# MOLAorg/mola_lidar_odometry

Hardware: AMD Instinct MI355X
Metric: scans/sec (KITTI 64-beam, ~120k pts, 1M-pt map) @1/2/4/8 GPU; ATE vs ref (higher is better)
Workload: dtype f32 points / f64 accumulators

## Files before the change

### mola_lidar_odometry_amd/csrc/mh_k_launch.h

```cpp
#pragma once

__global__ __launch_bounds__(kBlock, MH_QUAD_WAVES) void k_match4(const IcpDeviceState* __restrict__ st,
                                                   const float* __restrict__ lx, const float* __restrict__ ly,
                                                   const float* __restrict__ lz, uint32_t n, MapView map,
                                                   float4* __restrict__ pair_q, uint32_t* __restrict__ pair_gidx,
                                                   const uint32_t* __restrict__ perm
#ifdef MH_DEBUG_WAVETRACE
                                                   , unsigned long long* __restrict__ wtrace
#endif
) {
  k_match4_body(st, lx, ly, lz, n, map, pair_q, pair_gidx, perm
#ifdef MH_DEBUG_WAVETRACE
                , wtrace
#endif
  );
}
#ifndef MH_FLAT_WAVES
#define MH_FLAT_WAVES 6
#endif
#ifndef MH_FLAT_THREADS
#define MH_FLAT_THREADS 64
#endif
constexpr uint32_t kFlatThreads = MH_FLAT_THREADS;
constexpr uint32_t kFlatPointsPerBlock = kFlatThreads;
__device__ __forceinline__ uint32_t nblk_flat_dev(uint32_t n) { return (n + kFlatPointsPerBlock - 1u) / kFlatPointsPerBlock; }
constexpr uint32_t kFlatGridUnit = 8u;
inline uint32_t nblk_flat(size_t n) { return (uint32_t)(((n + kFlatPointsPerBlock - 1) / kFlatPointsPerBlock + kFlatGridUnit - 1) / kFlatGridUnit * kFlatGridUnit); }
__device__ __forceinline__ void k_match_flat_body(const IcpDeviceState* __restrict__ st, const float* __restrict__ lx,
                                                  const float* __restrict__ ly, const float* __restrict__ lz, uint32_t n,
                                                  MapView map, float4* __restrict__ pair_q, uint32_t* __restrict__ pair_gidx,
                                                  const uint32_t* __restrict__ perm, uint32_t block_x) {
  __shared__ FlatWave sh[kFlatThreads / 64];
  typedef const IcpDeviceState __attribute__((address_space(4))) * cstate_ptr;
  const cstate_ptr cst = (cstate_ptr)uniform_const_ptr(st);
  if (cst->done) return;
  const uint32_t bx = block_x;
  const uint32_t i0 = bx * kFlatPointsPerBlock + (threadIdx.x & ~63u);
  if (i0 >= n) return;
  const bool have_prev = cst->iter > 0 && !map.no_prev_bound;
  double T[12];
#pragma unroll
  for (int k = 0; k < 12; k++) T[k] = cst->T[k];
  match_flat_wave(sh[threadIdx.x >> 6], map, T, cst->cur_thr2, cst->cur_ang2, have_prev, lx, ly, lz, n, i0, pair_q, pair_gidx, perm);
}
__global__ __launch_bounds__(kFlatThreads, MH_FLAT_WAVES) void k_match_flat(const IcpDeviceState* __restrict__ st, const float* __restrict__ lx,
                                                             const float* __restrict__ ly, const float* __restrict__ lz, uint32_t n,
                                                             MapView map, float4* __restrict__ pair_q,
                                                             uint32_t* __restrict__ pair_gidx, const uint32_t* __restrict__ perm) {
  k_match_flat_body(st, lx, ly, lz, n, map, pair_q, pair_gidx, perm, blockIdx.x);
}
__global__ __launch_bounds__(kBlock, MH_QUAD_WAVES) void k_match4_b(const BatchJob* __restrict__ jobs) {
  const BatchJob& j = jobs[blockIdx.y];
  k_match4_body(j.st, j.lx, j.ly, j.lz, j.n, j.map, j.pair_q, j.pair_gidx, nullptr
#ifdef MH_DEBUG_WAVETRACE
                , nullptr
#endif
  );
}
__global__ __launch_bounds__(kFlatThreads, MH_FLAT_WAVES) void k_match_flat_b(const BatchJob* __restrict__ jobs) {
  uint32_t job = blockIdx.y, bx = blockIdx.x;
  const uint32_t whole = gridDim.y & ~7u;
  if (blockIdx.y < whole) {
    const uint32_t L = blockIdx.x + blockIdx.y * gridDim.x, xcd = L % 8u, slot = L / 8u;
    job = xcd + 8u * (slot / gridDim.x);
    bx = slot % gridDim.x;
  }
  const BatchJob& j = jobs[job];
  k_match_flat_body(j.st, j.lx, j.ly, j.lz, j.n, j.map, j.pair_q, j.pair_gidx, nullptr, bx);
}
#ifdef MH_DEV_VARIANTS
#include "mh_dev_variants.h"
#endif
template <bool SIGNED>
__global__ __launch_bounds__(kBlock, MH_ACCUM_WAVES) void k_accum(const IcpDeviceState* __restrict__ st, uint32_t first,
                                                  const MatchK* __restrict__ kp, const float* __restrict__ lx,
                                                  const float* __restrict__ ly, const float* __restrict__ lz, uint32_t n,
                                                  const float4* __restrict__ pair_q,
                                                  const uint32_t* __restrict__ pair_gidx, double* __restrict__ partials,
                                                  uint32_t pstride) {
  k_accum_body<SIGNED>(st, first, kp, lx, ly, lz, n, pair_q, pair_gidx, partials, pstride, blockIdx.x);
}
template <bool SIGNED>
__global__ __launch_bounds__(kBlock, MH_ACCUM_WAVES) void k_accum_b(const BatchJob* __restrict__ jobs, uint32_t first) {
  const BatchJob& j = jobs[blockIdx.y];
  const uint32_t bx = blockIdx.x;
  if (bx >= j.nba) return;
  k_accum_body<SIGNED>(j.st, first, j.mk, j.lx, j.ly, j.lz, j.n, j.pair_q, j.pair_gidx, j.part, j.nba, bx);
}
__global__ __launch_bounds__(kSolveThreads) void k_solve(IcpDeviceState* __restrict__ st, const SolveK* __restrict__ kp,
                                                         const double* __restrict__ partA, uint32_t nA, uint32_t strideA,
                                                         const double* __restrict__ partB, uint32_t nB,
                                                         uint32_t strideB, uint32_t first) {
  k_solve_body(st, kp, partA, nA, strideA, partB, nB, strideB, first);
}
__global__ __launch_bounds__(kSolveThreads) void k_solve_b(const BatchJob* __restrict__ jobs, uint32_t first) {
  const BatchJob& j = jobs[blockIdx.y];
  const uint32_t cols = first ? j.nbm : j.nba;
  k_solve_body(j.st, j.sk, j.part, cols, cols, nullptr, 0u, 0u, first);
}
__global__ void k_cov_prepare(IcpDeviceState* __restrict__ st, const SolveK* __restrict__ kp, uint32_t force) {
  k_cov_prepare_body(st, kp, force);
}
__global__ void k_cov_prepare_b(const BatchJob* __restrict__ jobs) {
  const BatchJob& j = jobs[blockIdx.y];
  k_cov_prepare_body(j.st, j.sk, 0u);
}
__global__ __launch_bounds__(kBlock) void k_cov_accum(const IcpDeviceState* __restrict__ st, uint32_t force,
                                                      const float* __restrict__ lx, const float* __restrict__ ly,
                                                      const float* __restrict__ lz, uint32_t n,
                                                      const uint32_t* __restrict__ pair_gidx,
                                                      double* __restrict__ partials, uint32_t pstride) {
  k_cov_accum_body(st, force, lx, ly, lz, n, pair_gidx, partials, pstride, blockIdx.x);
}
__global__ __launch_bounds__(kBlock) void k_cov_accum_b(const BatchJob* __restrict__ jobs) {
  const BatchJob& j = jobs[blockIdx.y];
  if (blockIdx.x >= j.nb) return;
  k_cov_accum_body(j.st, 0u, j.lx, j.ly, j.lz, j.n, j.pair_gidx, j.part, j.nb, blockIdx.x);
}
__global__ __launch_bounds__(kSolveThreads) void k_cov_finalize(IcpDeviceState* __restrict__ st, uint32_t force,
                                                                const double* __restrict__ partA, uint32_t nA,
                                                                uint32_t strideA, const double* __restrict__ partB,
                                                                uint32_t nB, uint32_t strideB) {
  k_cov_finalize_body(st, force, partA, nA, strideA, partB, nB, strideB);
}
__global__ __launch_bounds__(kSolveThreads) void k_cov_finalize_b(const BatchJob* __restrict__ jobs) {
  const BatchJob& j = jobs[blockIdx.y];
// ... 34 lines not shown
```

### mola_lidar_odometry_amd/csrc/mh_k_layers.h

```cpp
#pragma once

struct LayerDesc {
  MapView map;
  const float *lx, *ly, *lz;
  float4* pair_q;
  uint32_t* pair_gidx;
  MatchK mk;
  uint32_t n;
  uint32_t col_off;
  uint32_t cov_off;
  uint32_t run_from;
  uint32_t run_up_to;
  uint32_t kpp;
};

struct LayerTable {
  uint32_t n_pairs, pad;
  uint32_t blk_match[MH_MAX_LAYER_PAIRS + 1];
  uint32_t blk_acc[MH_MAX_LAYER_PAIRS + 1];
  uint32_t blk_cov[MH_MAX_LAYER_PAIRS + 1];
  LayerDesc d[MH_MAX_LAYER_PAIRS];
};

typedef const LayerTable __attribute__((address_space(4))) * clayers_ptr;

__device__ __forceinline__ uint32_t layer_of(const uint32_t __attribute__((address_space(4))) * start, uint32_t np, uint32_t b) {
  uint32_t li = 0;
  for (uint32_t k = 1; k < np; k++) li += b >= start[k] ? 1u : 0u;
  return li;
}

__device__ __forceinline__ bool layer_active(const clayers_ptr ct, uint32_t li, uint32_t iter) {
  const uint32_t from = ct->d[li].run_from, up_to = ct->d[li].run_up_to;
  return iter >= from && (up_to == 0u || iter <= up_to);
}

typedef const IcpDeviceState __attribute__((address_space(4))) * clayers_state_ptr;
__device__ __forceinline__ void match_layers_wave(FlatWave& sh, const clayers_state_ptr cst, const clayers_ptr ct, const uint32_t b) {
  const uint32_t li = layer_of(ct->blk_match, ct->n_pairs, b);
  const uint32_t n = ct->d[li].n;
  const uint32_t i0 = (b - ct->blk_match[li]) * kFlatPointsPerBlock + (threadIdx.x & ~63u);
  if (i0 >= n) return;
  const uint32_t iter = cst->iter;
  if (!layer_active(ct, li, iter)) {
    const uint32_t i = i0 + (uint32_t)__lane_id();
    if (i < n) {
      G(reinterpret_cast<f32x4*>(ct->d[li].pair_q))[i] = (f32x4){0.f, 0.f, 0.f, -__builtin_inff()};
      G(ct->d[li].pair_gidx)[i] = kNoMatch;
    }
    return;
  }
#ifdef MH_DEBUG_WAVETRACE
  static_assert(sizeof(MapView) == 56, "MapView changed: copy the new field in k_match_layers");
#else
  static_assert(sizeof(MapView) == 48, "MapView changed: copy the new field in k_match_layers");
#endif
  MapView map;
  map.slots = ct->d[li].map.slots;
  map.pts = ct->d[li].map.pts;
  map.mask = ct->d[li].map.mask;
  map.inv_vs = ct->d[li].map.inv_vs;
  map.vs = ct->d[li].map.vs;
  map.trunc = ct->d[li].map.trunc;
  map.ndt = ct->d[li].map.ndt;
  map.no_prev_bound = ct->d[li].map.no_prev_bound;
  map.pts_q = ct->d[li].map.pts_q;
#ifdef MH_DEBUG_WAVETRACE
  map.dbg_stop = ct->d[li].map.dbg_stop;
#endif
  const bool have_prev = iter > ct->d[li].run_from && !map.no_prev_bound;
  double T[12];
#pragma unroll
  for (int k = 0; k < 12; k++) T[k] = cst->T[k];
  const double thr = G(ct->d[li].mk.thr)[iter];
  const float thr2 = (float)(thr * thr);
  match_flat_wave(sh, map, T, thr2, ct->d[li].mk.ang2, have_prev, ct->d[li].lx, ct->d[li].ly, ct->d[li].lz, n, i0,
                  ct->d[li].pair_q, ct->d[li].pair_gidx, nullptr);
}

__global__ __launch_bounds__(kFlatThreads, MH_FLAT_WAVES) void k_match_layers(const IcpDeviceState* __restrict__ st,
                                                                               const LayerTable* __restrict__ tab) {
  __shared__ FlatWave sh[kFlatThreads / 64];
  const clayers_state_ptr cst = (clayers_state_ptr)uniform_const_ptr(st);
  if (cst->done) return;
  match_layers_wave(sh[threadIdx.x >> 6], cst, (clayers_ptr)uniform_const_ptr(tab), blockIdx.x);
}

__global__ __launch_bounds__(kBlock, MH_ACCUM_WAVES) void k_accum_layers(const IcpDeviceState* __restrict__ st,
                                                                         const LayerTable* __restrict__ tab, uint32_t first,
                                                                         double* __restrict__ partials, uint32_t pstride) {
  const clayers_ptr ct = (clayers_ptr)uniform_const_ptr(tab);
  const uint32_t li = layer_of(ct->blk_acc, ct->n_pairs, blockIdx.x);
  k_accum_body<true>(st, first, &tab->d[li].mk, ct->d[li].lx, ct->d[li].ly, ct->d[li].lz, ct->d[li].n, ct->d[li].pair_q,
                     ct->d[li].pair_gidx, partials + ct->d[li].col_off, pstride, blockIdx.x - ct->blk_acc[li]);
}

__global__ __launch_bounds__(kBlock) void k_cov_accum_layers(const IcpDeviceState* __restrict__ st,
                                                             const LayerTable* __restrict__ tab, double* __restrict__ partials,
                                                             uint32_t pstride) {
  const clayers_ptr ct = (clayers_ptr)uniform_const_ptr(tab);
  const uint32_t li = layer_of(ct->blk_cov, ct->n_pairs, blockIdx.x);
  k_cov_accum_body(st, 0u, ct->d[li].lx, ct->d[li].ly, ct->d[li].lz, ct->d[li].n, ct->d[li].pair_gidx,
                   partials + ct->d[li].cov_off, pstride, blockIdx.x - ct->blk_cov[li]);
}

struct LayerBatchJob {
  const LayerTable* tab;
  IcpDeviceState* st;
  double* part;
  uint32_t tot_acc, tot_cov;
};

struct LayerBatchTable {
  uint32_t n_jobs, pad;
  uint32_t job_blk_match[MH_MAX_LAYER_BATCH_JOBS + 1];
  uint32_t job_blk_acc[MH_MAX_LAYER_BATCH_JOBS + 1];
  uint32_t job_blk_cov[MH_MAX_LAYER_BATCH_JOBS + 1];
  LayerBatchJob j[MH_MAX_LAYER_BATCH_JOBS];
};

typedef const LayerBatchTable __attribute__((address_space(4))) * clayer_batch_ptr;

__global__ __launch_bounds__(kFlatThreads, MH_FLAT_WAVES) void k_match_layers_b(const LayerBatchTable* __restrict__ bt) {
  __shared__ FlatWave sh[kFlatThreads / 64];
  const clayer_batch_ptr cb = (clayer_batch_ptr)uniform_const_ptr(bt);
  const uint32_t ji = layer_of(cb->job_blk_match, cb->n_jobs, blockIdx.x);
  const clayers_state_ptr cst = (clayers_state_ptr)uniform_const_ptr(cb->j[ji].st);
  if (cst->done) return;
  match_layers_wave(sh[threadIdx.x >> 6], cst, (clayers_ptr)uniform_const_ptr(cb->j[ji].tab), blockIdx.x - cb->job_blk_match[ji]);
}

__global__ __launch_bounds__(kBlock, MH_ACCUM_WAVES) void k_accum_layers_b(const LayerBatchTable* __restrict__ bt, uint32_t first) {
  const clayer_batch_ptr cb = (clayer_batch_ptr)uniform_const_ptr(bt);
  const uint32_t ji = layer_of(cb->job_blk_acc, cb->n_jobs, blockIdx.x);
  const IcpDeviceState* const st = cb->j[ji].st;
  if (((clayers_state_ptr)uniform_const_ptr(st))->done) return;
  const LayerTable* const tab = cb->j[ji].tab;
  const clayers_ptr ct = (clayers_ptr)uniform_const_ptr(tab);
  const uint32_t b = blockIdx.x - cb->job_blk_acc[ji];
  const uint32_t li = layer_of(ct->blk_acc, ct->n_pairs, b);
  k_accum_body<true>(st, first, &tab->d[li].mk, ct->d[li].lx, ct->d[li].ly, ct->d[li].lz, ct->d[li].n, ct->d[li].pair_q,
                     ct->d[li].pair_gidx, cb->j[ji].part + ct->d[li].col_off, cb->j[ji].tot_acc, b - ct->blk_acc[li]);
}

__global__ __launch_bounds__(kBlock) void k_cov_accum_layers_b(const LayerBatchTable* __restrict__ bt) {
  const clayer_batch_ptr cb = (clayer_batch_ptr)uniform_const_ptr(bt);
  const uint32_t ji = layer_of(cb->job_blk_cov, cb->n_jobs, blockIdx.x);
  const clayers_ptr ct = (clayers_ptr)uniform_const_ptr(cb->j[ji].tab);
  const uint32_t b = blockIdx.x - cb->job_blk_cov[ji];
  const uint32_t li = layer_of(ct->blk_cov, ct->n_pairs, b);
  k_cov_accum_body(cb->j[ji].st, 0u, ct->d[li].lx, ct->d[li].ly, ct->d[li].lz, ct->d[li].n, ct->d[li].pair_gidx,
                   cb->j[ji].part + ct->d[li].cov_off, cb->j[ji].tot_cov, b - ct->blk_cov[li]);
}
```

### mola_lidar_odometry_amd/csrc/mh_k_match.h

```cpp
#pragma once

template <bool FUSED, int MODE >
__global__ __launch_bounds__(kBlock, MH_MATCH_WAVES) void k_match(const IcpDeviceState* __restrict__ st, PoseArg Targ, float thr2_arg,
                                                  uint32_t apply_thr, const MatchK* __restrict__ kp, const float* __restrict__ lx,
                                                  const float* __restrict__ ly, const float* __restrict__ lz, uint32_t n,
                                                  MapView map, float4* __restrict__ pair_q,
                                                  uint32_t* __restrict__ pair_gidx, double* __restrict__ partials,
                                                  uint32_t pstride) {
  __shared__ BlockSum<kAccN> lds;
  const MatchK k = *kp;
  double T[12];
  float thr2;
  double kparam = 0.0;
  if (FUSED) {
    if (st->done) return;
    const uint32_t it = st->iter;
#pragma unroll
    for (int i = 0; i < 12; i++) T[i] = st->T[i];
    const double thr = k.thr[it];
    thr2 = (float)(thr * thr);
    kparam = k.kparam[it];
  } else {
#pragma unroll
    for (int i = 0; i < 12; i++) T[i] = Targ.m[i];
// ... 81 lines not shown
        const double c = 1.0 / sqrt(t * t + 1.0), sn = t * c;
        const double app = A[p][p] - t * apq, aqq = A[q][q] + t * apq;
        const double arp = c * A[r][p] - sn * A[r][q], arq = sn * A[r][p] + c * A[r][q];
        A[p][p] = app; A[q][q] = aqq; A[p][q] = 0.0; A[q][p] = 0.0;
        A[r][p] = arp; A[p][r] = arp; A[r][q] = arq; A[q][r] = arq;
#pragma unroll
        for (int v = 0; v < 3; v++) {
          const double vip = c * V[v][p] - sn * V[v][q], viq = sn * V[v][p] + c * V[v][q];
          V[v][p] = vip; V[v][q] = viq;
        }
      }
    }
  }
  const double w0 = A[0][0], w1 = A[1][1], w2 = A[2][2];
  int imin = 0;
  double wmin = w0, wmax = w0;
  if (w1 < wmin) { wmin = w1; imin = 1; }
  if (w2 < wmin) { wmin = w2; imin = 2; }
  if (w1 > wmax) wmax = w1;
  if (w2 > wmax) wmax = w2;
  if (wmax > 0.0 && !(wmin > a.plane_eigen_threshold * wmax)) {
    double nv[3] = {imin == 0 ? V[0][0] : (imin == 1 ? V[0][1] : V[0][2]), imin == 0 ? V[1][0] : (imin == 1 ? V[1][1] : V[1][2]),
                    imin == 0 ? V[2][0] : (imin == 1 ? V[2][1] : V[2][2])};
    const double len = sqrt(nv[0] * nv[0] + nv[1] * nv[1] + nv[2] * nv[2]);
    int big = 0;
    if (fabs(nv[1]) > fabs(nv[big])) big = 1;
    if (fabs(nv[2]) > fabs(nv[big])) big = 2;
    const double sgn = ((big == 0 ? nv[0] : (big == 1 ? nv[1] : nv[2])) < 0.0 ? -1.0 : 1.0) / len;
    nv[0] *= sgn; nv[1] *= sgn; nv[2] *= sgn;
    const double dist = fabs((nv[0] * ((double)px - mu[0]) + nv[1] * ((double)py - mu[1])) + nv[2] * ((double)pz - mu[2]));
    if (!(dist > a.distance_threshold)) {
      rc = make_float4((float)mu[0], (float)mu[1], (float)mu[2], 1.f);
      rn = make_float4((float)nv[0], (float)nv[1], (float)nv[2], 0.f);
    }
  }
}
__global__ __launch_bounds__(kBlock) void k_match_pl_knn(PoseArg Targ, PlKnnArg a, const float* __restrict__ lx, const float* __restrict__ ly,
                                                         const float* __restrict__ lz, uint32_t n, MapView map, float4* __restrict__ pl_c,
                                                         float4* __restrict__ pl_n) {
  const uint32_t i = blockIdx.x * kBlock + threadIdx.x;
  if (i >= n) return;
  double T[12];
#pragma unroll
  for (int j = 0; j < 12; j++) T[j] = Targ.m[j];
  float px, py, pz;
  transform_point(T, lx[i], ly[i], lz[i], px, py, pz);
  float4 rc = make_float4(0.f, 0.f, 0.f, 0.f), rn = make_float4(0.f, 0.f, 0.f, 0.f);
  knnkey_t best[kMaxPlaneKnn];
  nn_search_kbest(map, px, py, pz, a.knn, best);
  uint32_t cnt = 0;
#pragma unroll
  for (int r = 0; r < kMaxPlaneKnn; r++) {
    const bool in = (uint32_t)r < a.knn && best[r] != ~0ull && __uint_as_float((uint32_t)(best[r] >> 32)) < a.radius2;
    cnt += (in && cnt == (uint32_t)r) ? 1u : 0u;
  }
  if (cnt >= a.min_pts) {
    const gpts_ptr pts4 = (gpts_ptr)map.pts;
    f32x4 nb[kMaxPlaneKnn];
#pragma unroll
    for (int r = 0; r < kMaxPlaneKnn; r++) nb[r] = pts4[(uint32_t)r < cnt ? (uint32_t)best[r] : (uint32_t)best[0]];
    pl_knn_plane(a, cnt, [&](int r) { return nb[r]; }, px, py, pz, rc, rn);
  }
  pl_c[i] = rc;
  pl_n[i] = rn;
}
__global__ void k_div_idx(uint32_t* __restrict__ idx, uint32_t n, uint32_t k) {
  const uint32_t i = blockIdx.x * blockDim.x + threadIdx.x;
  if (i < n) idx[i] /= k;
}

#ifdef MH_DEBUG_WAVETRACE
__device__ unsigned long long g_phase[32];
#define MH_PHASE(i) do { if (threadIdx.x == 0) g_phase[i] = wall_clock64(); } while (0)
extern "C" __attribute__((visibility("default"))) int mh_debug_phases(unsigned long long* host_out) {
  (void)hipDeviceSynchronize();
  return hipMemcpyFromSymbol(host_out, HIP_SYMBOL(g_phase), sizeof(g_phase)) == hipSuccess ? 0 : 2;
}
extern "C" __attribute__((visibility("default"))) int mh_debug_flat_counters(unsigned long long* host_out, int reset) {
  (void)hipDeviceSynchronize();
  if (hipMemcpyFromSymbol(host_out, HIP_SYMBOL(mh::g_flatdbg), sizeof(mh::g_flatdbg)) != hipSuccess) return 2;
  if (reset) { unsigned long long z[16] = {0}; (void)hipMemcpyToSymbol(HIP_SYMBOL(mh::g_flatdbg), z, sizeof(z)); }
  return 0;
}
#define MH_LOOP_STAMPS unsigned long long lp_t = wall_clock64(), lp_acc[12] = {0, 0, 0, 0, 0, 0, 0, 0, 0, 0, 0, 0}
#define MH_LOOP_STAMP(i) do { const unsigned long long now_ = wall_clock64(); lp_acc[i] += now_ - lp_t; lp_t = now_; } while (0)
#define MH_LOOP_STAMPS_OUT(steps) do { if (blockIdx.x == 0 && threadIdx.x == 0) { for (int q_ = 0; q_ < 12; q_++) g_phase[16 + q_] = lp_acc[q_]; g_phase[28] = (steps); } } while (0)
#else
#define MH_PHASE(i) do { } while (0)
#define MH_LOOP_STAMPS do { } while (0)
#define MH_LOOP_STAMP(i) do { } while (0)
#define MH_LOOP_STAMPS_OUT(steps) do { } while (0)
#endif
#ifdef MH_DEBUG_WAVETRACE
static unsigned long long* g_wtrace = nullptr;
extern "C" __attribute__((visibility("default"))) int mh_debug_wavetrace(unsigned long long* host_out, size_t n_waves) {
  if (!g_wtrace) { if (hipMalloc(&g_wtrace, 16u << 20) != hipSuccess) return 1; (void)hipMemset(g_wtrace, 0, 16u << 20); return 0; }
  (void)hipDeviceSynchronize();
  return hipMemcpy(host_out, g_wtrace, n_waves * 16, hipMemcpyDeviceToHost) == hipSuccess ? 0 : 2;
}
#endif
__device__ __forceinline__ void k_match4_body(const IcpDeviceState* __restrict__ st,
                                                   const float* __restrict__ lx, const float* __restrict__ ly,
                                                   const float* __restrict__ lz, uint32_t n, MapView map,
                                                   float4* __restrict__ pair_q, uint32_t* __restrict__ pair_gidx,
                                                   const uint32_t* __restrict__ perm
#ifdef MH_DEBUG_WAVETRACE
                                                   , unsigned long long* __restrict__ wtrace
#endif
) {
#ifdef MH_DEBUG_WAVETRACE
  struct WT { unsigned long long* p; unsigned long long t0; uint32_t w;
              __device__ ~WT() { if ((threadIdx.x & 63) == 0 && p) { p[2 * w] = t0; p[2 * w + 1] = wall_clock64(); } } }
      wt{wtrace, (unsigned long long)wall_clock64(), (blockIdx.x * kBlock + threadIdx.x) >> 6};
#endif
  const uint32_t gl = blockIdx.x * kBlock + threadIdx.x;
  const uint32_t i = gl >> 2, sub = gl & 3u;
  const uint32_t ic = i < n ? i : n - 1;
  const uint32_t o = perm ? G(perm)[ic] : ic;
  const float x = G(lx)[ic], y = G(ly)[ic], z = G(lz)[ic];
  typedef const IcpDeviceState __attribute__((address_space(4))) * cstate_ptr;
  const cstate_ptr cst = (cstate_ptr)uniform_const_ptr(st);
  const uint32_t done = cst->done;
  const bool have_prev = cst->iter > 0 && !map.no_prev_bound;
  f32x4 prev = (f32x4){0.f, 0.f, 0.f, __builtin_inff()};
  if (have_prev) prev = G(reinterpret_cast<const f32x4*>(pair_q))[o];
  double T[12];
#pragma unroll
  for (int k = 0; k < 12; k++) T[k] = cst->T[k];
  const float thr2 = cst->cur_thr2, ang2 = cst->cur_ang2;
  if (done) return;
  if (i >= n) return;
  float px, py, pz;
  transform_point(T, x, y, z, px, py, pz);
  float bound0 = __builtin_inff();
  if (prev.w < __builtin_inff()) {
    const float dx = prev.x - px, dy = prev.y - py, dz = prev.z - pz;
    bound0 = (dx * dx + dy * dy) + dz * dz;
  }
  const NNResult r = nn_search_quad(map, sub, px, py, pz, bound0);
  if (sub == 0) {
    const float n2 = (px * px + py * py) + pz * pz;
    const bool ok = r.found && (r.d2 < thr2 + ang2 * n2);
    G(reinterpret_cast<f32x4*>(pair_q))[o] = (f32x4){r.pt.x, r.pt.y, r.pt.z, r.d2};
    G(pair_gidx)[o] = ok ? __float_as_uint(r.pt.w) : kNoMatch;
  }
}

constexpr uint32_t kFused16MaxPoints = 12288;
constexpr uint32_t kRowMaxPoints = 32768;
```

### mola_lidar_odometry_amd/csrc/mh_nn_flat.h

```cpp
#pragma once
#include "mh_nn_device.h"

namespace mh {

constexpr int kFlatLPP = 4;
#ifndef MH_FLAT_W
#define MH_FLAT_W 8
#endif
#ifndef MH_FLAT_PROBES
#define MH_FLAT_PROBES 4
#endif
constexpr int kFlatProbes = MH_FLAT_PROBES;
constexpr int kFlatW = MH_FLAT_W;
constexpr int kFlatMaxCand = 8;
#ifndef MH_FLAT_CHUNKS
#define MH_FLAT_CHUNKS 768
#endif
constexpr int kFlatMaxChunks = MH_FLAT_CHUNKS;
constexpr uint32_t kFlatMaxRecords = 1u << 30;

template <int MAXC, int NCL, int NCH>
struct FlatWaveT {
  static constexpr int kMaxCand = MAXC;
  static constexpr int kCands = NCL;
  static constexpr int kMaxChunks = NCH;
  f32x4 P[64];
  unsigned long long KB[64];
  unsigned long long RES[64];
  uint32_t CH[NCH];
  unsigned short CL[NCL];
  unsigned char CHP[NCH];
  unsigned char SLOWF[64];
  unsigned char SL[64];
  uint32_t NCH_, NVALID;
};
typedef FlatWaveT<kFlatMaxCand, 64 * kFlatMaxCand, kFlatMaxChunks> FlatWave;
#ifndef MH_LW_NCL
#define MH_LW_NCL 1024
#endif
#ifndef MH_LW_NCH
#define MH_LW_NCH 1024
#endif
typedef FlatWaveT<27, MH_LW_NCL, MH_LW_NCH> FlatWaveSmall;

__device__ __forceinline__ uint32_t lanes_below(unsigned long long m) {
  return __builtin_amdgcn_mbcnt_hi((uint32_t)(m >> 32), __builtin_amdgcn_mbcnt_lo((uint32_t)m, 0u));
}

struct FlatInsertMin {
  template <class FW>
  __device__ __forceinline__ void operator()(FW& sh, uint32_t p, unsigned long long key) const {
    (void)__hip_atomic_fetch_min(&sh.RES[p], key, __ATOMIC_RELAXED, __HIP_MEMORY_SCOPE_WORKGROUP);
  }
};
template <class FW, class INS = FlatInsertMin>
__device__ __forceinline__ uint32_t flat_plan_scan(FW& sh, const MapView& m, uint32_t lane, uint32_t cmask, unsigned long long kbase,
                                                   float px, float py, float pz, float b0, unsigned long long init,
                                                   const INS ins = INS()) {
  constexpr int kFlatMaxCand = FW::kMaxCand;
  constexpr int kFlatMaxChunks = FW::kMaxChunks;
  const gslots_ptr slots4 = (gslots_ptr)m.slots;
  const gpts_ptr spts = (gpts_ptr)m.pts_q;
  uint32_t n_cands;
  const uint32_t ncand = (uint32_t)__builtin_popcount(cmask);
  const uint32_t cincl = wave_scan_incl(ncand);
  n_cands = (uint32_t)__builtin_amdgcn_readlane((int)cincl, 63);
  sh.P[lane] = (f32x4){px, py, pz, b0};
  uint32_t nvalid = 0;
  if (n_cands) {
    sh.KB[lane] = kbase;
    sh.RES[lane] = init;
    sh.SLOWF[lane] = 0;
    if (lane == 0) { sh.NCH_ = 0; sh.NVALID = (uint32_t)kFlatMaxChunks; }
    {
      uint32_t mm = cmask, at = cincl - ncand;
      if (kFlatMaxCand <= 8) {
#pragma unroll
        for (int j = 0; j < (kFlatMaxCand <= 8 ? kFlatMaxCand : 1); j++) {
          if (mm) {
            const uint32_t code = (uint32_t)__builtin_ctz(mm);
            mm &= mm - 1;
            sh.CL[at + (uint32_t)j] = (unsigned short)(lane | (code << 8));
          }
        }
      } else {
        while (mm) {
          const uint32_t code = (uint32_t)__builtin_ctz(mm);
          mm &= mm - 1;
          sh.CL[at++] = (unsigned short)(lane | (code << 8));
        }
      }
    }
    wave_sync_lds_nn();
    uint32_t nch_total = 0;
    for (uint32_t base = 0; base < n_cands; base += 64u * (uint32_t)kFlatProbes) {
      uint32_t ent[kFlatProbes];
      unsigned long long keys[kFlatProbes];
      u32x4 sls[kFlatProbes];
#pragma unroll
      for (int k = 0; k < kFlatProbes; k++) {
        const uint32_t c = base + 64u * (uint32_t)k + lane;
        ent[k] = sh.CL[c < n_cands ? c : 0u];
        keys[k] = nn_key_of(sh.KB[ent[k] & 63u], (int)(ent[k] >> 8));
        sls[k] = slots4[hash_key(keys[k]) & m.mask];
      }
#pragma unroll
      for (int k = 0; k < kFlatProbes; k++) {
        if (base + 64u * (uint32_t)k >= n_cands) break;
        const uint32_t c = base + 64u * (uint32_t)k + lane;
        const bool act = c < n_cands;
        const uint32_t p = ent[k] & 63u;
        const int code = (int)(ent[k] >> 8);
        const f32x4 P = sh.P[p];
        uint32_t f, cnt, qv;
        nn_resolve(m, slots4, keys[k], sls[k], act, f, cnt, &qv);
        quad_narrow(m, qv, code, P.x, P.y, P.w, f, cnt);
        const uint32_t nchunks = (cnt + (uint32_t)kFlatLPP - 1u) / (uint32_t)kFlatLPP;
        const uint32_t incl = wave_scan_incl(nchunks);
        const uint32_t pos = nch_total + incl - nchunks;
        nch_total += (uint32_t)__builtin_amdgcn_readlane((int)incl, 63);
        if (nchunks) {
          if (pos + nchunks > (uint32_t)kFlatMaxChunks) {
            sh.SLOWF[p] = 1;
            (void)__hip_atomic_fetch_min(&sh.NVALID, pos, __ATOMIC_RELAXED, __HIP_MEMORY_SCOPE_WORKGROUP);
          } else {
#pragma unroll 1
            for (uint32_t j = 0; j < nchunks; j++) {
              const uint32_t rem = cnt - (uint32_t)kFlatLPP * j;
              sh.CH[pos + j] = (f + (uint32_t)kFlatLPP * j) | (((rem < (uint32_t)kFlatLPP ? rem : (uint32_t)kFlatLPP) - 1u) << 30);
              sh.CHP[pos + j] = (unsigned char)p;
            }
          }
        }
      }
    }
    wave_sync_lds_nn();
    {
      const uint32_t a = nch_total;
      const uint32_t b = sh.NVALID;
      nvalid = (uint32_t)__builtin_amdgcn_readfirstlane((int)(a < b ? a : b));
    }
    const uint32_t grp = lane >> 2, sub = lane & 3u;
    for (uint32_t t0 = 0; t0 < nvalid; t0 += 16u * (uint32_t)kFlatW) {
      f32x4 rec[kFlatW];
      uint32_t pp[kFlatW];
      bool valid[kFlatW];
#pragma unroll
      for (int u = 0; u < kFlatW; u++) {
        const uint32_t t = t0 + 16u * (uint32_t)u + grp;
        const bool ok = t < nvalid;
        const uint32_t tt = ok ? t : 0u;
        const uint32_t ch = sh.CH[tt];
        pp[u] = sh.CHP[tt];
        const uint32_t last = ch >> 30;
        valid[u] = ok && sub <= last;
        rec[u] = spts[(ch & 0x3FFFFFFFu) + (sub < last ? sub : last)];
      }
#pragma unroll
      for (int u = 0; u < kFlatW; u++) {
        const f32x4 Pq = sh.P[pp[u]];
        const float dx = rec[u].x - Pq.x, dy = rec[u].y - Pq.y, dz = rec[u].z - Pq.z;
        const float d2 = (dx * dx + dy * dy) + dz * dz;
        if (valid[u] && d2 <= Pq.w) ins(sh, pp[u], ((unsigned long long)__float_as_uint(d2) << 32) | __float_as_uint(rec[u].w));
      }
    }
    wave_sync_lds_nn();
  }
  return n_cands;
}

__device__ __forceinline__ float flat_signed_d2(float d2, bool accepted) {
  return __uint_as_float(__float_as_uint(d2) | (accepted ? 0u : 0x80000000u));
}
__device__ __forceinline__ void match_flat_wave(FlatWave& sh, const MapView& m, const double* __restrict__ T, float thr2,
                                                float ang2, bool have_prev, const float* __restrict__ lx,
                                                const float* __restrict__ ly, const float* __restrict__ lz, uint32_t n,
                                                uint32_t i0, float4* __restrict__ pair_q, uint32_t* __restrict__ pair_gidx,
                                                const uint32_t* __restrict__ perm) {
  const uint32_t lane = (uint32_t)__lane_id();
  const uint32_t i = i0 + lane;
  const bool in = i < n;
  const uint32_t ic = in ? i : n - 1;
  const uint32_t o = perm ? G(perm)[ic] : ic;
  const gslots_ptr slots4 = (gslots_ptr)m.slots;
  const gpts_ptr pts4 = (gpts_ptr)m.pts;
  const gpts_ptr spts = (gpts_ptr)m.pts_q;
  const float x = G(lx)[ic], y = G(ly)[ic], z = G(lz)[ic];
  f32x4 prev = (f32x4){0.f, 0.f, 0.f, __builtin_inff()};
  if (have_prev) prev = G(reinterpret_cast<const f32x4*>(pair_q))[o];
  float px, py, pz;
  transform_point(T, x, y, z, px, py, pz);
  float b0 = __builtin_inff();
  if (fabsf(prev.w) < __builtin_inff()) {
    const float dx = prev.x - px, dy = prev.y - py, dz = prev.z - pz;
    b0 = (dx * dx + dy * dy) + dz * dz;
  }
  const float lim = 1.0e6f;
  const bool okrange = ((int)(fabsf(px * m.inv_vs) < lim) & (int)(fabsf(py * m.inv_vs) < lim) & (int)(fabsf(pz * m.inv_vs) < lim)) != 0;
  const bool unbounded = in && okrange && !(b0 < __builtin_inff());
  bool own_done = false;
  unsigned long long res0 = 0;
  bool planned = false;
  uint32_t n_cands = 0;
  const int cx = voxel_of(px, m.inv_vs, m.trunc), cy = voxel_of(py, m.inv_vs, m.trunc), cz = voxel_of(pz, m.inv_vs, m.trunc);
  const unsigned long long kbase = pack_key(cx - 1, cy - 1, cz - 1);
  if (__ballot(unbounded) != 0ull) {
    n_cands = flat_plan_scan(sh, m, lane, unbounded ? (1u << 13) : 0u, kbase, px, py, pz, b0, 0x7F800000FFFFFFFFull);
    const unsigned long long r0 = sh.RES[lane];
    if (unbounded && (uint32_t)r0 != 0xFFFFFFFFu && sh.SLOWF[lane] == 0) {
      own_done = true;
      res0 = r0;
      b0 = __uint_as_float((uint32_t)(r0 >> 32));
    }
    wave_sync_lds_nn();
  }
  uint32_t cmask = 0;
  planned = in && okrange && b0 < __builtin_inff();
  if (__ballot(planned) != 0ull) {
    const Gaps gx = axis_gaps(px, cx, m.vs, m.trunc), gy = axis_gaps(py, cy, m.vs, m.trunc), gz = axis_gaps(pz, cz, m.vs, m.trunc);
    cmask = 1u << 13;
    const float fx = fmaxf(gx.s[0], gx.s[2]), fy = fmaxf(gy.s[0], gy.s[2]), fz = fmaxf(gz.s[0], gz.s[2]);
    const bool far_dead = (fx * 0.9999f > b0) && (fy * 0.9999f > b0) && (fz * 0.9999f > b0);
    if (__ballot(planned && !far_dead) == 0ull) {
      const bool xl = gx.s[0] <= gx.s[2], yl = gy.s[0] <= gy.s[2], zl = gz.s[0] <= gz.s[2];
      const float nx = xl ? gx.s[0] : gx.s[2], ny = yl ? gy.s[0] : gy.s[2], nz = zl ? gz.s[0] : gz.s[2];
      const uint32_t cx_ = xl ? 4u : 22u, cy_ = yl ? 10u : 16u, cz_ = zl ? 12u : 14u;
      const uint32_t dx_ = cx_ - 13u, dy_ = cy_ - 13u;
      const float lxy = nx + ny;
      cmask |= (!(nx * 0.9999f > b0)) ? (1u << cx_) : 0u;
      cmask |= (!(ny * 0.9999f > b0)) ? (1u << cy_) : 0u;
      cmask |= (!(nz * 0.9999f > b0)) ? (1u << cz_) : 0u;
      cmask |= (!(lxy * 0.9999f > b0)) ? (1u << (cy_ + dx_)) : 0u;
      cmask |= (!((nx + nz) * 0.9999f > b0)) ? (1u << (cz_ + dx_)) : 0u;
      cmask |= (!((ny + nz) * 0.9999f > b0)) ? (1u << (cz_ + dy_)) : 0u;
      cmask |= (!((lxy + nz) * 0.9999f > b0)) ? (1u << (cz_ + dx_ + dy_)) : 0u;
    } else {
#pragma unroll
      for (int c = 0; c < 27; c++) {
        if (c == 13) continue;
        const int ix = c / 9, iy = (c / 3) % 3, iz = c % 3;
        const float sx = ix == 1 ? 0.f : gx.s[ix], sy = iy == 1 ? 0.f : gy.s[iy], sz = iz == 1 ? 0.f : gz.s[iz];
        const float lb = ((sx + sy) + sz) * 0.9999f;
        cmask |= (!(lb > b0)) ? (1u << c) : 0u;
      }
    }
    if (!planned) cmask = 0;
    if (own_done) cmask &= ~(1u << 13);
    if (__builtin_popcount(cmask) > kFlatMaxCand) {
      planned = false;
      cmask = 0;
    }
  }
  n_cands = flat_plan_scan(sh, m, lane, cmask, kbase, px, py, pz, b0,
                           own_done ? res0 : (((unsigned long long)__float_as_uint(b0) << 32) | 0xFFFFFFFFull));
  bool slow = in && !planned;
  float b0s = b0;
  {
    unsigned long long res = own_done ? res0 : 0xFFFFFFFFFFFFFFFFull;
    bool spilled = false;
    if (n_cands) {
      res = sh.RES[lane];
      spilled = sh.SLOWF[lane] != 0;
    }
    const uint32_t idx = (uint32_t)res;
    if (planned && !spilled && idx != 0xFFFFFFFFu) {
      const f32x4 w = pts4[idx];
      const float d2 = __uint_as_float((uint32_t)(res >> 32));
      const float n2 = (px * px + py * py) + pz * pz;
      const bool ok = d2 < thr2 + ang2 * n2;
      G(reinterpret_cast<f32x4*>(pair_q))[o] = (f32x4){w.x, w.y, w.z, flat_signed_d2(d2, ok)};
      G(pair_gidx)[o] = ok ? __float_as_uint(w.w) : kNoMatch;
    } else if (planned) {
      slow = true;
      if (!spilled) b0s = __builtin_inff();
    }
  }
  const unsigned long long sm = __ballot(slow);
  if (sm == 0ull) return;
  const uint32_t ns = (uint32_t)__builtin_popcountll(sm);
  wave_sync_lds_nn();
  if (slow) {
    sh.SL[lanes_below(sm)] = (unsigned char)lane;
    sh.P[lane] = (f32x4){px, py, pz, b0s};
  }
  wave_sync_lds_nn();
  const uint32_t grp = lane >> 2, sub = lane & 3u;
  for (uint32_t g = 0; g < ns; g += 16u) {
    const uint32_t k = g + grp;
    if (k < ns) {
      const uint32_t p = sh.SL[k];
      const f32x4 P = sh.P[p];
      const NNResult r = nn_search_quad(m, sub, P.x, P.y, P.z, P.w);
      if (sub == 0u) {
        const uint32_t ip = i0 + p;
        const uint32_t op = perm ? G(perm)[ip] : ip;
        const float n2 = (P.x * P.x + P.y * P.y) + P.z * P.z;
        const bool ok = r.found && (r.d2 < thr2 + ang2 * n2);
        G(reinterpret_cast<f32x4*>(pair_q))[op] = (f32x4){r.pt.x, r.pt.y, r.pt.z, flat_signed_d2(r.d2, ok)};
        G(pair_gidx)[op] = ok ? __float_as_uint(r.pt.w) : kNoMatch;
      }
    }
  }
}


#ifdef MH_DEBUG_WAVETRACE
static __device__ unsigned long long g_flatdbg[16];
#define MH_FLATDBG(i, v) do { const unsigned long long b_ = __ballot(v); if (lane == 0 && b_) atomicAdd(&g_flatdbg[i], (unsigned long long)__builtin_popcountll(b_)); } while (0)
#define MH_FLATDBG_ADD(i, v) do { if (lane == 0) atomicAdd(&g_flatdbg[i], (unsigned long long)(v)); } while (0)
#else
#define MH_FLATDBG(i, v) do { } while (0)
#define MH_FLATDBG_ADD(i, v) do { } while (0)
#endif
struct FlatHit {
  f32x4 pt;
  float d2;
  bool found;
};
template <class FW>
__device__ __forceinline__ FlatHit flat_search_points(FW& sh, const MapView& m, bool in, float px, float py, float pz, float b0) {
  constexpr int kFlatMaxCand = FW::kMaxCand;
  const uint32_t lane = (uint32_t)__lane_id();
  const gpts_ptr pts4 = (gpts_ptr)m.pts;
  const float lim = 1.0e6f;
  const bool okrange = ((int)(fabsf(px * m.inv_vs) < lim) & (int)(fabsf(py * m.inv_vs) < lim) & (int)(fabsf(pz * m.inv_vs) < lim)) != 0;
  const bool unbounded = in && okrange && !(b0 < __builtin_inff());
  bool own_empty = false;
  MH_FLATDBG_ADD(0, 1);
  MH_FLATDBG(1, in);
  MH_FLATDBG(2, unbounded);
  bool own_done = false;
  unsigned long long res0 = 0;
  bool planned = false;
  uint32_t n_cands = 0;
  const int cx = voxel_of(px, m.inv_vs, m.trunc), cy = voxel_of(py, m.inv_vs, m.trunc), cz = voxel_of(pz, m.inv_vs, m.trunc);
  const unsigned long long kbase = pack_key(cx - 1, cy - 1, cz - 1);
  if (__ballot(unbounded) != 0ull) {
    n_cands = flat_plan_scan(sh, m, lane, unbounded ? (1u << 13) : 0u, kbase, px, py, pz, b0, 0x7F800000FFFFFFFFull);
    const unsigned long long r0 = sh.RES[lane];
    if (unbounded && (uint32_t)r0 != 0xFFFFFFFFu && sh.SLOWF[lane] == 0) {
      own_done = true;
      res0 = r0;
      b0 = __uint_as_float((uint32_t)(r0 >> 32));
    } else if (unbounded && sh.SLOWF[lane] == 0 && kFlatMaxCand >= 27) {
      own_empty = true;
    }
    wave_sync_lds_nn();
  }
  uint32_t cmask = 0;
  planned = in && okrange && (b0 < __builtin_inff() || own_empty);
  MH_FLATDBG(3, in && !planned);
  if (__ballot(planned) != 0ull) {
    const Gaps gx = axis_gaps(px, cx, m.vs, m.trunc), gy = axis_gaps(py, cy, m.vs, m.trunc), gz = axis_gaps(pz, cz, m.vs, m.trunc);
    cmask = 1u << 13;
    const float fx = fmaxf(gx.s[0], gx.s[2]), fy = fmaxf(gy.s[0], gy.s[2]), fz = fmaxf(gz.s[0], gz.s[2]);
    const bool far_dead = (fx * 0.9999f > b0) && (fy * 0.9999f > b0) && (fz * 0.9999f > b0);
    if (__ballot(planned && !far_dead) == 0ull) {
      const bool xl = gx.s[0] <= gx.s[2], yl = gy.s[0] <= gy.s[2], zl = gz.s[0] <= gz.s[2];
      const float nx = xl ? gx.s[0] : gx.s[2], ny = yl ? gy.s[0] : gy.s[2], nz = zl ? gz.s[0] : gz.s[2];
      const uint32_t cx_ = xl ? 4u : 22u, cy_ = yl ? 10u : 16u, cz_ = zl ? 12u : 14u;
      const uint32_t dx_ = cx_ - 13u, dy_ = cy_ - 13u;
      const float lxy = nx + ny;
      cmask |= (!(nx * 0.9999f > b0)) ? (1u << cx_) : 0u;
      cmask |= (!(ny * 0.9999f > b0)) ? (1u << cy_) : 0u;
      cmask |= (!(nz * 0.9999f > b0)) ? (1u << cz_) : 0u;
      cmask |= (!(lxy * 0.9999f > b0)) ? (1u << (cy_ + dx_)) : 0u;
      cmask |= (!((nx + nz) * 0.9999f > b0)) ? (1u << (cz_ + dx_)) : 0u;
      cmask |= (!((ny + nz) * 0.9999f > b0)) ? (1u << (cz_ + dy_)) : 0u;
      cmask |= (!((lxy + nz) * 0.9999f > b0)) ? (1u << (cz_ + dx_ + dy_)) : 0u;
    } else {
#pragma unroll
      for (int c = 0; c < 27; c++) {
        if (c == 13) continue;
        const int ix = c / 9, iy = (c / 3) % 3, iz = c % 3;
        const float sx = ix == 1 ? 0.f : gx.s[ix], sy = iy == 1 ? 0.f : gy.s[iy], sz = iz == 1 ? 0.f : gz.s[iz];
        const float lb = ((sx + sy) + sz) * 0.9999f;
        cmask |= (!(lb > b0)) ? (1u << c) : 0u;
      }
    }
    if (!planned) cmask = 0;
    if (own_done || own_empty) cmask &= ~(1u << 13);
    MH_FLATDBG(4, __builtin_popcount(cmask) > kFlatMaxCand);
    if (__builtin_popcount(cmask) > kFlatMaxCand) {
      planned = false;
      cmask = 0;
    }
  }
  n_cands = flat_plan_scan(sh, m, lane, cmask, kbase, px, py, pz, b0,
                           own_done ? res0 : (((unsigned long long)__float_as_uint(b0) << 32) | 0xFFFFFFFFull));
  MH_FLATDBG_ADD(7, n_cands);
  FlatHit h;
  h.pt = (f32x4)(0.f);
  h.d2 = __builtin_inff();
  h.found = false;
  bool slow = in && !planned;
  float b0s = b0;
// ... 57 lines not shown
```

Baseline: 6843.

## Process oversized neighbour-cell masks in multiple flat passes instead of slow path

In the flat wave matcher, lanes whose 26-neighbour candidate mask exceeds the per-pass candidate cap are no longer sent to the slow quad NN search. They are handled in extra plan/scan passes that pick face cells first, then edges and corners, and prune the remaining cells against the updated best distance after each pass. Lanes whose own voxel is empty but in range are now planned too, and emit a no-match result directly when nothing is found. The aim is to keep more points on the fast LDS-planned path and avoid the serial slow search, at the cost of loop overhead, extra LDS syncs and register pressure in the multi-pass kernel. Debug counters are also added behind the wavetrace flag.

```diff
diff --git a/mola_lidar_odometry_amd/csrc/mh_k_launch.h b/mola_lidar_odometry_amd/csrc/mh_k_launch.h
--- a/mola_lidar_odometry_amd/csrc/mh_k_launch.h
+++ b/mola_lidar_odometry_amd/csrc/mh_k_launch.h
@@ -41,7 +41,13 @@
   double T[12];
 #pragma unroll
   for (int k = 0; k < 12; k++) T[k] = cst->T[k];
-  match_flat_wave(sh[threadIdx.x >> 6], map, T, cst->cur_thr2, cst->cur_ang2, have_prev, lx, ly, lz, n, i0, pair_q, pair_gidx, perm);
+#ifdef MH_FLAT_SINGLE_PASS
+  constexpr bool kPasses = false;
+#else
+  constexpr bool kPasses = true;
+#endif
+  match_flat_wave<kPasses>(sh[threadIdx.x >> 6], map, T, cst->cur_thr2, cst->cur_ang2, have_prev, lx, ly, lz, n, i0, pair_q, pair_gidx,
+                           perm MH_FLATMW_PASS(cst->iter));
 }
 __global__ __launch_bounds__(kFlatThreads, MH_FLAT_WAVES) void k_match_flat(const IcpDeviceState* __restrict__ st, const float* __restrict__ lx,
                                                              const float* __restrict__ ly, const float* __restrict__ lz, uint32_t n,
diff --git a/mola_lidar_odometry_amd/csrc/mh_k_layers.h b/mola_lidar_odometry_amd/csrc/mh_k_layers.h
--- a/mola_lidar_odometry_amd/csrc/mh_k_layers.h
+++ b/mola_lidar_odometry_amd/csrc/mh_k_layers.h
@@ -74,8 +74,8 @@
   for (int k = 0; k < 12; k++) T[k] = cst->T[k];
   const double thr = G(ct->d[li].mk.thr)[iter];
   const float thr2 = (float)(thr * thr);
-  match_flat_wave(sh, map, T, thr2, ct->d[li].mk.ang2, have_prev, ct->d[li].lx, ct->d[li].ly, ct->d[li].lz, n, i0,
-                  ct->d[li].pair_q, ct->d[li].pair_gidx, nullptr);
+  match_flat_wave<false>(sh, map, T, thr2, ct->d[li].mk.ang2, have_prev, ct->d[li].lx, ct->d[li].ly, ct->d[li].lz, n, i0,
+                         ct->d[li].pair_q, ct->d[li].pair_gidx, nullptr);
 }
 
 __global__ __launch_bounds__(kFlatThreads, MH_FLAT_WAVES) void k_match_layers(const IcpDeviceState* __restrict__ st,
diff --git a/mola_lidar_odometry_amd/csrc/mh_k_match.h b/mola_lidar_odometry_amd/csrc/mh_k_match.h
--- a/mola_lidar_odometry_amd/csrc/mh_k_match.h
+++ b/mola_lidar_odometry_amd/csrc/mh_k_match.h
@@ -187,6 +187,12 @@
   if (reset) { unsigned long long z[16] = {0}; (void)hipMemcpyToSymbol(HIP_SYMBOL(mh::g_flatdbg), z, sizeof(z)); }
   return 0;
 }
+extern "C" __attribute__((visibility("default"))) int mh_debug_flat_wave_counters(unsigned long long* host_out, int reset) {
+  (void)hipDeviceSynchronize();
+  if (hipMemcpyFromSymbol(host_out, HIP_SYMBOL(mh::g_flatmw), sizeof(mh::g_flatmw)) != hipSuccess) return 2;
+  if (reset) { static unsigned long long z[32 * 16]; (void)hipMemcpyToSymbol(HIP_SYMBOL(mh::g_flatmw), z, sizeof(z)); }
+  return 0;
+}
 #define MH_LOOP_STAMPS unsigned long long lp_t = wall_clock64(), lp_acc[12] = {0, 0, 0, 0, 0, 0, 0, 0, 0, 0, 0, 0}
 #define MH_LOOP_STAMP(i) do { const unsigned long long now_ = wall_clock64(); lp_acc[i] += now_ - lp_t; lp_t = now_; } while (0)
 #define MH_LOOP_STAMPS_OUT(steps) do { if (blockIdx.x == 0 && threadIdx.x == 0) { for (int q_ = 0; q_ < 12; q_++) g_phase[16 + q_] = lp_acc[q_]; g_phase[28] = (steps); } } while (0)
diff --git a/mola_lidar_odometry_amd/csrc/mh_nn_flat.h b/mola_lidar_odometry_amd/csrc/mh_nn_flat.h
--- a/mola_lidar_odometry_amd/csrc/mh_nn_flat.h
+++ b/mola_lidar_odometry_amd/csrc/mh_nn_flat.h
@@ -13,6 +13,7 @@
 constexpr int kFlatProbes = MH_FLAT_PROBES;
 constexpr int kFlatW = MH_FLAT_W;
 constexpr int kFlatMaxCand = 8;
+constexpr int kFlatPasses = (27 + kFlatMaxCand - 1) / kFlatMaxCand + 1;
 #ifndef MH_FLAT_CHUNKS
 #define MH_FLAT_CHUNKS 768
 #endif
@@ -35,6 +36,7 @@
   uint32_t NCH_, NVALID;
 };
 typedef FlatWaveT<kFlatMaxCand, 64 * kFlatMaxCand, kFlatMaxChunks> FlatWave;
+static_assert(MH_FLAT_CHUNKS != 768 || sizeof(FlatWave) <= 7168, "FlatWave: 7 KB per wave is what 5.5 waves per SIMD cost; a pass never emits more than 64 x kFlatMaxCand candidates");
 #ifndef MH_LW_NCL
 #define MH_LW_NCL 1024
 #endif
@@ -172,11 +174,60 @@
 __device__ __forceinline__ float flat_signed_d2(float d2, bool accepted) {
   return __uint_as_float(__float_as_uint(d2) | (accepted ? 0u : 0x80000000u));
 }
+#ifdef MH_DEBUG_WAVETRACE
+static __device__ unsigned long long g_flatdbg[16];
+#define MH_FLATDBG(i, v) do { const unsigned long long b_ = __ballot(v); if (lane == 0 && b_) atomicAdd(&g_flatdbg[i], (unsigned long long)__builtin_popcountll(b_)); } while (0)
+#define MH_FLATDBG_ADD(i, v) do { if (lane == 0) atomicAdd(&g_flatdbg[i], (unsigned long long)(v)); } while (0)
+static __device__ unsigned long long g_flatmw[32][16];
+#define MH_FLATMW(i, v) do { const unsigned long long b_ = __ballot(v); if (lane == 0 && b_) atomicAdd(&g_flatmw[dbg_it < 31u ? dbg_it : 31u][i], (unsigned long long)__builtin_popcountll(b_)); } while (0)
+#define MH_FLATMW_ADD(i, v) do { if (lane == 0) atomicAdd(&g_flatmw[dbg_it < 31u ? dbg_it : 31u][i], (unsigned long long)(v)); } while (0)
+#define MH_FLATMW_ARG , uint32_t dbg_it = 31u
+#define MH_FLATMW_PASS(it) , (it)
+#else
+#define MH_FLATMW(i, v) do { } while (0)
+#define MH_FLATMW_ADD(i, v) do { } while (0)
+#define MH_FLATMW_ARG
+#define MH_FLATMW_PASS(it)
+#define MH_FLATDBG(i, v) do { } while (0)
+#define MH_FLATDBG_ADD(i, v) do { } while (0)
+#endif
+__device__ __forceinline__ uint32_t flat_mask26(const Gaps& gx, const Gaps& gy, const Gaps& gz, float b0) {
+  uint32_t mask = 0;
+#pragma unroll
+  for (int c = 0; c < 27; c++) {
+    if (c == 13) continue;
+    const int ix = c / 9, iy = (c / 3) % 3, iz = c % 3;
+    const float sx = ix == 1 ? 0.f : gx.s[ix], sy = iy == 1 ? 0.f : gy.s[iy], sz = iz == 1 ? 0.f : gz.s[iz];
+    const float lb = ((sx + sy) + sz) * 0.9999f;
+    mask |= (!(lb > b0)) ? (1u << c) : 0u;
+  }
+  return mask;
+}
+constexpr uint32_t kFlatOwn = 1u << 13;
+constexpr uint32_t kFlatFaces = (1u << 4) | (1u << 10) | (1u << 12) | (1u << 14) | (1u << 16) | (1u << 22);
+constexpr uint32_t kFlatCorners = (1u << 0) | (1u << 2) | (1u << 6) | (1u << 8) | (1u << 18) | (1u << 20) | (1u << 24) | (1u << 26);
+constexpr uint32_t kFlatEdges = 0x07FFFFFFu & ~(kFlatOwn | kFlatFaces | kFlatCorners);
+__device__ __forceinline__ uint32_t flat_pick(uint32_t mask) {
+  if (__builtin_popcount(mask) <= kFlatMaxCand) return mask;
+  uint32_t sel = mask & (kFlatOwn | kFlatFaces);
+  uint32_t outer = mask & kFlatEdges, corners = mask & kFlatCorners;
+#pragma unroll
+  for (int j = 0; j < kFlatMaxCand; j++) {
+    if (__builtin_popcount(sel) < kFlatMaxCand) {
+      if (outer == 0u) { outer = corners; corners = 0u; }
+      const uint32_t low = outer & (0u - outer);
+      sel |= low;
+      outer ^= low;
+    }
+  }
+  return sel;
+}
+template <bool PASSES = true>
 __device__ __forceinline__ void match_flat_wave(FlatWave& sh, const MapView& m, const double* __restrict__ T, float thr2,
                                                 float ang2, bool have_prev, const float* __restrict__ lx,
                                                 const float* __restrict__ ly, const float* __restrict__ lz, uint32_t n,
                                                 uint32_t i0, float4* __restrict__ pair_q, uint32_t* __restrict__ pair_gidx,
-                                                const uint32_t* __restrict__ perm) {
+                                                const uint32_t* __restrict__ perm MH_FLATMW_ARG) {
   const uint32_t lane = (uint32_t)__lane_id();
   const uint32_t i = i0 + lane;
   const bool in = i < n;
@@ -198,7 +249,11 @@
   const float lim = 1.0e6f;
   const bool okrange = ((int)(fabsf(px * m.inv_vs) < lim) & (int)(fabsf(py * m.inv_vs) < lim) & (int)(fabsf(pz * m.inv_vs) < lim)) != 0;
   const bool unbounded = in && okrange && !(b0 < __builtin_inff());
+  MH_FLATMW_ADD(0, 1);
+  MH_FLATMW(1, in);
+  MH_FLATMW(2, unbounded);
   bool own_done = false;
+  bool own_empty = false;
   unsigned long long res0 = 0;
   bool planned = false;
   uint32_t n_cands = 0;
@@ -211,11 +266,18 @@
       own_done = true;
       res0 = r0;
       b0 = __uint_as_float((uint32_t)(r0 >> 32));
+    } else if (PASSES && unbounded && sh.SLOWF[lane] == 0) {
+      own_empty = true;
     }
     wave_sync_lds_nn();
   }
   uint32_t cmask = 0;
-  planned = in && okrange && b0 < __builtin_inff();
+  uint32_t rest = 0;
+  bool spilled0 = false;
+  unsigned long long bigm = 0;
+  planned = in && okrange && (b0 < __builtin_inff() || own_empty);
+  MH_FLATMW(3, in && !planned);
+  MH_FLATMW(9, own_empty);
   if (__ballot(planned) != 0ull) {
     const Gaps gx = axis_gaps(px, cx, m.vs, m.trunc), gy = axis_gaps(py, cy, m.vs, m.trunc), gz = axis_gaps(pz, cz, m.vs, m.trunc);
     cmask = 1u << 13;
@@ -245,24 +307,70 @@
       }
     }
     if (!planned) cmask = 0;
-    if (own_done) cmask &= ~(1u << 13);
-    if (__builtin_popcount(cmask) > kFlatMaxCand) {
+    if (own_done || own_empty) cmask &= ~(1u << 13);
+    MH_FLATMW(4, __builtin_popcount(cmask) > kFlatMaxCand);
+    if (PASSES) {
+      bigm = __ballot(__builtin_popcount(cmask) > kFlatMaxCand);
+      if (bigm != 0ull) {
+        const uint32_t sel = flat_pick(cmask);
+        rest = cmask & ~sel;
+        cmask = sel;
+      }
+    } else if (__builtin_popcount(cmask) > kFlatMaxCand) {
       planned = false;
       cmask = 0;
     }
   }
   n_cands = flat_plan_scan(sh, m, lane, cmask, kbase, px, py, pz, b0,
                            own_done ? res0 : (((unsigned long long)__float_as_uint(b0) << 32) | 0xFFFFFFFFull));
+  MH_FLATMW_ADD(11, n_cands);
+  if (PASSES && bigm != 0ull) {
+    unsigned long long kb = 0;
+    float qx = 0.f, qy = 0.f, qz = 0.f;
+#pragma unroll 1
+    for (int pass = 1; pass < kFlatPasses; pass++) {
+      {
+        const unsigned long long r = sh.RES[lane];
+        kb = sh.KB[lane];
+        const f32x4 Pl = sh.P[lane];
+        qx = Pl.x, qy = Pl.y, qz = Pl.z;
+        if (sh.SLOWF[lane] != 0) {
+          spilled0 = true;
+          rest = 0;
+        } else if ((uint32_t)r != 0xFFFFFFFFu) {
+          own_done = true;
+          res0 = r;
+          b0 = __uint_as_float((uint32_t)(r >> 32));
+        }
+      }
+      {
+        const Gaps gx = axis_gaps(qx, voxel_of(qx, m.inv_vs, m.trunc), m.vs, m.trunc), gy = axis_gaps(qy, voxel_of(qy, m.inv_vs, m.trunc), m.vs, m.trunc),
+                   gz = axis_gaps(qz, voxel_of(qz, m.inv_vs, m.trunc), m.vs, m.trunc);
+        rest &= flat_mask26(gx, gy, gz, b0);
+      }
+      if (__ballot(rest != 0u) == 0ull) break;
+      wave_sync_lds_nn();
+      const uint32_t sel = flat_pick(rest);
+      rest &= ~sel;
+      n_cands = flat_plan_scan(sh, m, lane, sel, kb, qx, qy, qz, b0,
+                               own_done ? res0 : (((unsigned long long)__float_as_uint(b0) << 32) | 0xFFFFFFFFull));
+      MH_FLATMW_ADD(8, 1);
+      MH_FLATMW_ADD(11, n_cands);
+    }
+    const f32x4 Pl = sh.P[lane];
+    px = Pl.x, py = Pl.y, pz = Pl.z;
+  }
   bool slow = in && !planned;
   float b0s = b0;
   {
     unsigned long long res = own_done ? res0 : 0xFFFFFFFFFFFFFFFFull;
-    bool spilled = false;
+    bool spilled = PASSES && spilled0;
     if (n_cands) {
       res = sh.RES[lane];
-      spilled = sh.SLOWF[lane] != 0;
+      spilled = spilled || sh.SLOWF[lane] != 0;
     }
     const uint32_t idx = (uint32_t)res;
+    bool again = false, none = false;
     if (planned && !spilled && idx != 0xFFFFFFFFu) {
       const f32x4 w = pts4[idx];
       const float d2 = __uint_as_float((uint32_t)(res >> 32));
@@ -270,14 +378,25 @@
       const bool ok = d2 < thr2 + ang2 * n2;
       G(reinterpret_cast<f32x4*>(pair_q))[o] = (f32x4){w.x, w.y, w.z, flat_signed_d2(d2, ok)};
       G(pair_gidx)[o] = ok ? __float_as_uint(w.w) : kNoMatch;
+    } else if (PASSES && planned && own_empty && !spilled) {
+      G(reinterpret_cast<f32x4*>(pair_q))[o] = (f32x4){0.f, 0.f, 0.f, flat_signed_d2(__builtin_inff(), false)};
+      G(pair_gidx)[o] = kNoMatch;
+      none = true;
     } else if (planned) {
       slow = true;
+      again = true;
       if (!spilled) b0s = __builtin_inff();
     }
+    MH_FLATMW(5, again && spilled);
+    MH_FLATMW(6, again && !spilled);
+    MH_FLATMW(10, none);
+    (void)again;
+    (void)none;
   }
   const unsigned long long sm = __ballot(slow);
   if (sm == 0ull) return;
   const uint32_t ns = (uint32_t)__builtin_popcountll(sm);
+  MH_FLATMW_ADD(7, ns);
   wave_sync_lds_nn();
   if (slow) {
     sh.SL[lanes_below(sm)] = (unsigned char)lane;
@@ -304,14 +423,6 @@
 }
 
 
-#ifdef MH_DEBUG_WAVETRACE
-static __device__ unsigned long long g_flatdbg[16];
-#define MH_FLATDBG(i, v) do { const unsigned long long b_ = __ballot(v); if (lane == 0 && b_) atomicAdd(&g_flatdbg[i], (unsigned long long)__builtin_popcountll(b_)); } while (0)
-#define MH_FLATDBG_ADD(i, v) do { if (lane == 0) atomicAdd(&g_flatdbg[i], (unsigned long long)(v)); } while (0)
-#else
-#define MH_FLATDBG(i, v) do { } while (0)
-#define MH_FLATDBG_ADD(i, v) do { } while (0)
-#endif
 struct FlatHit {
   f32x4 pt;
   float d2;
```

After: 6822. About the same (-0.3%).
